# rodrigo-paganini/kalman-vae

Hardware: AMD Instinct MI355X
Metric: sequences/sec (ELBO training step, 32x32xT bouncing-ball) (higher is better)
Workload: dtype f32; 1 GPU; BASELINE configs[1] (configs[2] per-GPU shard): bouncing-ball 32x32, T=50, batch=256/GPU, dynamics=lstm K=3, z=4, u=4, a=2, full train step (fwd incl. sigmoid(x_logits) + loss incl. active-unit stats + bwd + clip + Adam); both the GPU leg and the cpu_baseline leg do this work; preset=c2, global_batch=256, seq_len=50, parallelism=dp1, capture=hipgraph, loss_finite=True, dist_backend=none

## Files before the change

### kalman-vae_amd/csrc/kvae_vae.hip

```cpp
#include <hip/hip_runtime.h>

#include <stdint.h>
#include <stdio.h>
#include <stdlib.h>
#include <string.h>

#include "../../include/kvae_lgssm.h"

namespace kvae {}
using namespace kvae;

extern "C" int kvae_launch_status(const char *what);
static int launch_status(const char *what) { return kvae_launch_status(what); }

#include "vae_epilogue.h"

__device__ __forceinline__ void colsum_v4_body(const float *__restrict__ partials, float *__restrict__ out, int64_t rows, int64_t cols,
                                               unsigned block) {
  __shared__ float4 red[8][64];
  const int lane = threadIdx.x & 63, wv = threadIdx.x >> 6;
  const int64_t c = ((int64_t)block * 64 + lane) * 4;
  float4 s0 = make_float4(0.f, 0.f, 0.f, 0.f), s1 = s0, s2 = s0, s3 = s0;
  if (c < cols) {
    const float *p = partials + c;
// ... 193 lines not shown
}

constexpr int CA_BLOCKS = 512;
constexpr int CA_MAX_SEG = 1024;
__global__ __launch_bounds__(256) void k_grad_sumsq(const float *__restrict__ g, int64_t n, const int32_t *__restrict__ seg_of,
                                                    int n_seg, const float *__restrict__ seg_active,
                                                    const float *__restrict__ div_dev, float *__restrict__ seg_steps,
                                                    float *__restrict__ ws) {
  __shared__ float red[256];
  const float inv = div_dev ? 1.0f / fmaxf(*div_dev, 1.0f) : 1.0f;
  const bool gated = seg_of && seg_active;
  float s = 0.f;
  for (int64_t i = (int64_t)blockIdx.x * 256 + threadIdx.x; i < n; i += (int64_t)gridDim.x * 256) {
    float v = g[i] * inv;
    if (gated && seg_active[seg_of[i]] == 0.f) v = 0.f;
    s = fmaf(v, v, s);
  }
  red[threadIdx.x] = s;
  __syncthreads();
  for (int o = 128; o > 0; o >>= 1) {
    if ((int)threadIdx.x < o) red[threadIdx.x] += red[threadIdx.x + o];
    __syncthreads();
  }
  if (threadIdx.x == 0) ws[blockIdx.x] = red[0];
  if (blockIdx.x == 0)
    for (int sg = threadIdx.x; sg < n_seg; sg += 256)
      if (!seg_active || seg_active[sg] != 0.f) seg_steps[sg] += 1.0f;
}
__global__ __launch_bounds__(256) void k_clip_adam(float *__restrict__ p, const float *__restrict__ g, float *__restrict__ m,
                                                   float *__restrict__ v, int64_t n, const int32_t *__restrict__ seg_of, int n_seg,
                                                   const float *__restrict__ seg_active, const float *__restrict__ seg_steps,
                                                   const float *__restrict__ lr_dev, float lr, float beta1, float beta2, float eps,
                                                   float wd, float clip, const float *__restrict__ div_dev,
                                                   float *__restrict__ norm_out, const float *__restrict__ ws, int nparts) {
  __shared__ float red[256];
  __shared__ float s_step_size[CA_MAX_SEG], s_bc2s[CA_MAX_SEG];
  float s = 0.f;
  for (int i = threadIdx.x; i < nparts; i += 256) s += ws[i];
  red[threadIdx.x] = s;
  const float lrv = lr_dev ? *lr_dev : lr;
  for (int sg = threadIdx.x; sg < n_seg; sg += 256) {
    const float step = seg_steps[sg];
    const bool on = !seg_active || seg_active[sg] != 0.f;
    s_step_size[sg] = on ? lrv / (1.0f - powf(beta1, step)) : -1.0f;
    s_bc2s[sg] = on ? sqrtf(1.0f - powf(beta2, step)) : 1.0f;
  }
  __syncthreads();
  for (int o = 128; o > 0; o >>= 1) {
    if ((int)threadIdx.x < o) red[threadIdx.x] += red[threadIdx.x + o];
    __syncthreads();
  }
  const float total = sqrtf(red[0]);
  if (norm_out && blockIdx.x == 0 && threadIdx.x == 0) *norm_out = total;
  const float inv = div_dev ? 1.0f / fmaxf(*div_dev, 1.0f) : 1.0f;
  const float scale = inv * (clip > 0.f ? fminf(clip / (total + 1e-6f), 1.0f) : 1.0f);
  for (int64_t i = (int64_t)blockIdx.x * 256 + threadIdx.x; i < n; i += (int64_t)gridDim.x * 256) {
    const int sg = seg_of ? seg_of[i] : 0;
    const float step_size = s_step_size[sg], bc2s = s_bc2s[sg];
    if (step_size < 0.f) continue;
    float gi = g[i] * scale;
    const float pi = p[i];
    if (wd != 0.f) gi = fmaf(wd, pi, gi);
    const float mi = m[i] + (gi - m[i]) * (1.0f - beta1);
    const float vi = beta2 * v[i] + (1.0f - beta2) * gi * gi;
    m[i] = mi, v[i] = vi;
    p[i] = pi - step_size * mi / (sqrtf(vi) / bc2s + eps);
  }
}
extern "C" int kvae_clip_adam(float *params, const float *grads, float *exp_avg, float *exp_avg_sq, int64_t n,
                              const int32_t *seg_of, int32_t n_seg, const float *seg_active, float *seg_steps, const float *lr_dev,
                              float lr, float beta1, float beta2, float eps, float weight_decay, float clip, const float *div_dev,
                              float *norm_out, float *ws, void *stream) {
  if (!params || !grads || !exp_avg || !exp_avg_sq || !seg_steps || !ws) return KVAE_ERR_NULL;
  if (n < 1 || n_seg < 1 || n_seg > CA_MAX_SEG || (!seg_of && n_seg != 1)) return KVAE_ERR_ARG;
  const int64_t want = (n + 1023) / 1024;
  const unsigned parts = (unsigned)(want < CA_BLOCKS ? want : CA_BLOCKS);
  k_grad_sumsq<<<dim3(parts), dim3(256), 0, (hipStream_t)stream>>>(grads, n, seg_of, n_seg, seg_active, div_dev, seg_steps, ws);
  int rc = launch_status("k_grad_sumsq");
  if (rc) return rc;
  const unsigned blocks = (unsigned)((n + 255) / 256 < 2048 ? (n + 255) / 256 : 2048);
  k_clip_adam<<<dim3(blocks), dim3(256), 0, (hipStream_t)stream>>>(params, grads, exp_avg, exp_avg_sq, n, seg_of, n_seg, seg_active,
                                                                   seg_steps, lr_dev, lr, beta1, beta2, eps, weight_decay, clip,
                                                                   div_dev, norm_out, ws, (int)parts);
  return launch_status("k_clip_adam");
}

#include "vae_loss.h"

__global__ __launch_bounds__(256) void k_vae_bce_fwd(const float *__restrict__ logits, const float *__restrict__ x,
                                                     float *__restrict__ frame_ll, int64_t frames, int pixels) {
  const int64_t f = (int64_t)blockIdx.x * 4 + (threadIdx.x >> 6);
  const int lane = threadIdx.x & 63;
  if (f >= frames) return;
  const float *l = logits + f * pixels, *t = x + f * pixels;
  float acc = 0.f;
  if ((pixels & 3) == 0 && (((uintptr_t)l | (uintptr_t)t) & 15) == 0) {
    for (int i = lane * 4; i < pixels; i += 256) {
      const float4 a = *reinterpret_cast<const float4 *>(l + i), b = *reinterpret_cast<const float4 *>(t + i);
      acc += bce_logit(a.x, b.x) + bce_logit(a.y, b.y) + bce_logit(a.z, b.z) + bce_logit(a.w, b.w);
    }
  } else {
    for (int i = lane; i < pixels; i += 64) acc += bce_logit(l[i], t[i]);
  }
  for (int off = 32; off > 0; off >>= 1) acc += __shfl_down(acc, off, 64);
  if (lane == 0) frame_ll[f] = -acc;
}

__global__ __launch_bounds__(256) void k_vae_bce_bwd(const float *__restrict__ logits, const float *__restrict__ x,
                                                     const float *__restrict__ g_frame, float *__restrict__ g_logits,
                                                     int64_t total, int pixels) {
  for (int64_t i = ((int64_t)blockIdx.x * 256 + threadIdx.x) * 4; i < total; i += (int64_t)gridDim.x * 1024) {
    const float g = -g_frame[i / pixels];
    const float4 a = *reinterpret_cast<const float4 *>(logits + i), b = *reinterpret_cast<const float4 *>(x + i);
    *reinterpret_cast<float4 *>(g_logits + i) = make_float4(g * (sigmoid_stable(a.x) - b.x), g * (sigmoid_stable(a.y) - b.y),
                                                            g * (sigmoid_stable(a.z) - b.z), g * (sigmoid_stable(a.w) - b.w));
  }
}
__global__ __launch_bounds__(256) void k_vae_bce_bwd_scalar(const float *logits, const float *x, const float *g_frame,
                                                            float *g_logits, int64_t total, int pixels) {
  for (int64_t i = (int64_t)blockIdx.x * 256 + threadIdx.x; i < total; i += (int64_t)gridDim.x * 256)
    g_logits[i] = -g_frame[i / pixels] * (sigmoid_stable(logits[i]) - x[i]);
}

extern "C" {
int kvae_bce_frames_fwd(const float *logits, const float *x, float *frame_ll, int64_t frames, int32_t pixels, void *stream) {
  if (!logits || !x || !frame_ll) return KVAE_ERR_NULL;
  if (frames < 1 || pixels < 1) return KVAE_ERR_ARG;
  k_vae_bce_fwd<<<dim3((unsigned)((frames + 3) / 4)), dim3(256), 0, (hipStream_t)stream>>>(logits, x, frame_ll, frames, pixels);
  return launch_status("k_vae_bce_fwd");
}
int kvae_bce_frames_bwd(const float *logits, const float *x, const float *g_frame, float *g_logits, int64_t frames,
                        int32_t pixels, void *stream) {
  if (!logits || !x || !g_frame || !g_logits) return KVAE_ERR_NULL;
  if (frames < 1 || pixels < 1) return KVAE_ERR_ARG;
  const int64_t total = frames * pixels;
  const bool v4 = (pixels & 3) == 0 && ((((uintptr_t)logits | (uintptr_t)x | (uintptr_t)g_logits) & 15) == 0);
  if (v4)
    k_vae_bce_bwd<<<dim3(epi_grid(total / 4)), dim3(256), 0, (hipStream_t)stream>>>(logits, x, g_frame, g_logits, total, pixels);
  else
    k_vae_bce_bwd_scalar<<<dim3(epi_grid(total)), dim3(256), 0, (hipStream_t)stream>>>(logits, x, g_frame, g_logits, total, pixels);
  return launch_status("k_vae_bce_bwd");
}
}

#include "vae_conv_edge.h"
extern "C" {
int64_t kvae_conv_edge_partial_rows(int64_t N) { return N < 1024 ? (N < 1 ? 1 : N) : 1024; }

int kvae_dec_head_fwd(const float *in, const float *W, const float *bias, float *logits, float *w_scratch, int64_t N,
                      int32_t Cin, int32_t side, void *stream) {
  if (!in || !W || !bias || !logits || !w_scratch) return KVAE_ERR_NULL;
  if (N < 1) return KVAE_ERR_ARG;
  if (Cin != DH_CI || side != DH_S) return KVAE_ERR_DIMS;
  k_dec_head_prep<<<dim3(1), dim3(256), 0, (hipStream_t)stream>>>(W, w_scratch);
  k_dec_head_fwd<<<dim3((unsigned)N), dim3(256), 0, (hipStream_t)stream>>>(in, w_scratch, bias, logits);
  return launch_status("k_dec_head_fwd");
}
int kvae_dec_head_bwd(const float *in, const float *W, const float *g_logits, float *g_in, float *w_partials,
                      float *b_partials, float *w_scratch, int64_t N, int32_t Cin, int32_t side, void *stream) {
  if (!in || !W || !g_logits || !w_partials || !b_partials || !w_scratch) return KVAE_ERR_NULL;
  if (N < 1) return KVAE_ERR_ARG;
  if (Cin != DH_CI || side != DH_S) return KVAE_ERR_DIMS;
  if (g_in) {
    k_dec_head_prep<<<dim3(1), dim3(256), 0, (hipStream_t)stream>>>(W, w_scratch);
    k_dec_head_bwd_data<<<dim3((unsigned)N), dim3(256), 0, (hipStream_t)stream>>>(g_logits, w_scratch, g_in);
    const int rc = launch_status("k_dec_head_bwd_data");
    if (rc) return rc;
  }
  k_dec_head_wrw<<<dim3((unsigned)kvae_conv_edge_partial_rows(N)), dim3(256), 0, (hipStream_t)stream>>>(in, g_logits, w_partials,
                                                                                                     b_partials, N);
  return launch_status("k_dec_head_wrw");
}
int kvae_enc_stem_fwd(const float *x, const float *W, const float *bias, float *out, uint32_t *relu_bits, int64_t N, int32_t Cout,
                      int32_t side, void *stream) {
  if (!x || !W || !bias || !out) return KVAE_ERR_NULL;
  if (N < 1) return KVAE_ERR_ARG;
  if (Cout != ES_CO || side != ES_IN) return KVAE_ERR_DIMS;
  k_enc_stem_fwd<<<dim3((unsigned)N), dim3(256), 0, (hipStream_t)stream>>>(x, W, bias, out, relu_bits);
  return launch_status("k_enc_stem_fwd");
}
int kvae_enc_stem_bwd(const float *x, const float *out, const uint32_t *relu_bits, const float *g_out, float *w_partials,
                      float *b_partials, int64_t N, int32_t Cout, int32_t side, void *stream) {
  if (!x || (!out && !relu_bits) || !g_out || !w_partials || !b_partials) return KVAE_ERR_NULL;
  if (N < 1) return KVAE_ERR_ARG;
  if (Cout != ES_CO || side != ES_IN) return KVAE_ERR_DIMS;
  static const int mfma = getenv("KVAE_STEM_MFMA") ? atoi(getenv("KVAE_STEM_MFMA")) : 1;
  const dim3 grid((unsigned)kvae_conv_edge_partial_rows(N));
  if (mfma == 1 && relu_bits) k_enc_stem_wrw_mfma<true><<<grid, dim3(256), 0, (hipStream_t)stream>>>(x, out, relu_bits, g_out, w_partials, b_partials, N);
  else if (!out) return KVAE_ERR_NULL;
  else if (mfma) k_enc_stem_wrw_mfma<false><<<grid, dim3(256), 0, (hipStream_t)stream>>>(x, out, relu_bits, g_out, w_partials, b_partials, N);
  else k_enc_stem_wrw<<<grid, dim3(256), 0, (hipStream_t)stream>>>(x, out, g_out, w_partials, b_partials, N);
  return launch_status("k_enc_stem_wrw");
}
}

#include "vae_conv_mid.h"
static inline int64_t enc_mid_grid(int64_t N, int32_t side) {
  const int64_t fpi = side == 16 ? 2 : 8, iters = (N + fpi - 1) / fpi;
  return iters < 256 ? (iters < 1 ? 1 : iters) : 256;
}
extern "C" {
int64_t kvae_enc_mid_partial_rows(int64_t N, int32_t side) { return enc_mid_grid(N, side); }

int kvae_enc_mid_fwd(const float *in, const float *W, const float *bias, float *out, int64_t N, int32_t C, int32_t side,
                     void *stream) {
  if (!in || !W || !bias || !out) return KVAE_ERR_NULL;
  if (N < 1 || (N + 256 * 8) * EM_C * side * side * 4 >= EM_MAX_BYTES) return KVAE_ERR_ARG;
  if (C != EM_C || (side != 16 && side != 8)) return KVAE_ERR_DIMS;
  const dim3 grid((unsigned)enc_mid_grid(N, side));
  if (side == 16) k_enc_mid_fwd<16><<<grid, dim3(256), 0, (hipStream_t)stream>>>(in, W, bias, out, N);
  else k_enc_mid_fwd<8><<<grid, dim3(256), 0, (hipStream_t)stream>>>(in, W, bias, out, N);
  return launch_status("k_enc_mid_fwd");
}
int kvae_enc_mid_bwd(const float *in, const float *W, const float *out, const float *g_out, float *g_in,
                     float *w_partials, float *b_partials, int64_t N, int32_t C, int32_t side, void *stream) {
  if (!in || !W || !out || !g_out || !w_partials || !b_partials) return KVAE_ERR_NULL;
  if (N < 1 || (N + 256 * 8) * EM_C * side * side * 4 >= EM_MAX_BYTES) return KVAE_ERR_ARG;
  if (C != EM_C || (side != 16 && side != 8)) return KVAE_ERR_DIMS;
  const dim3 grid((unsigned)enc_mid_grid(N, side));
  if (g_in) {
    if (side == 16) k_enc_mid_bwd_data<16><<<grid, dim3(256), 0, (hipStream_t)stream>>>(W, out, g_out, g_in, N);
    else k_enc_mid_bwd_data<8><<<grid, dim3(256), 0, (hipStream_t)stream>>>(W, out, g_out, g_in, N);
    const int rc = launch_status("k_enc_mid_bwd_data");
    if (rc) return rc;
  }
  if (side == 16) k_enc_mid_wrw<16><<<grid, dim3(256), 0, (hipStream_t)stream>>>(in, out, g_out, w_partials, b_partials, N);
  else k_enc_mid_wrw<8><<<grid, dim3(256), 0, (hipStream_t)stream>>>(in, out, g_out, w_partials, b_partials, N);
  return launch_status("k_enc_mid_wrw");
}
}

#include "vae_conv_up_wino.h"
static bool dec_up_wino() {
  static const int env = getenv("KVAE_WINO") ? atoi(getenv("KVAE_WINO")) : 1;
  return env != 0;
}
static int g_dec_up_wgs = 0;
static inline int64_t dec_up_cap() {
  static const int env = getenv("KVAE_UP_WGS") ? atoi(getenv("KVAE_UP_WGS")) : 0;
  const int v = env >= 1 && env <= 256 ? env : __atomic_load_n(&g_dec_up_wgs, __ATOMIC_RELAXED);
  return v >= 1 && v <= 256 ? v : 256;
}
static inline int64_t dec_up_grid(int64_t N, int32_t side) {
  const int64_t fpi = side == 8 ? 2 : 8, iters = (N + fpi - 1) / fpi, cap = dec_up_cap();
  return iters < cap ? (iters < 1 ? 1 : iters) : cap;
}
extern "C" {
int64_t kvae_dec_up_partial_rows(int64_t N, int32_t side) { return dec_up_grid(N, side); }
int32_t kvae_dec_up_set_workgroups(int32_t n) {
  const int32_t prev = (int32_t)dec_up_cap();
  __atomic_store_n(&g_dec_up_wgs, n >= 1 && n <= 256 ? n : 0, __ATOMIC_RELAXED);
  return prev;
}

int kvae_dec_up_fwd(const float *x, const float *W, const float *bias, float *out, int64_t N, int32_t Cin, int32_t side,
                    void *stream) {
  if (!x || !W || !bias || !out) return KVAE_ERR_NULL;
  if (N < 1 || (N + 256 * 8) * UP_CO * side * side * 4 >= EM_MAX_BYTES) return KVAE_ERR_ARG;
  if (Cin != UP_CI || (side != 8 && side != 4)) return KVAE_ERR_DIMS;
  const dim3 grid((unsigned)dec_up_grid(N, side));
  if (dec_up_wino()) {
    const int64_t sets = side == 8 ? N : (N + 3) / 4;
    const dim3 wgrid((unsigned)(sets < dec_up_cap() ? sets : dec_up_cap()));
    if (side == 8) k_dec_up_fwd_wino<8><<<wgrid, dim3(512), 0, (hipStream_t)stream>>>(x, W, bias, out, N);
    else k_dec_up_fwd_wino<4><<<wgrid, dim3(512), 0, (hipStream_t)stream>>>(x, W, bias, out, N);
    return launch_status("k_dec_up_fwd_wino");
  }
  if (side == 8) k_dec_up_fwd<8><<<grid, dim3(256), 0, (hipStream_t)stream>>>(x, W, bias, out, N);
  else k_dec_up_fwd<4><<<grid, dim3(256), 0, (hipStream_t)stream>>>(x, W, bias, out, N);
  return launch_status("k_dec_up_fwd");
}
int kvae_dec_up_bwd(const float *x, const float *W, const float *out, const float *g_out, float *g_x, float *w_partials,
                    float *b_partials, int64_t N, int32_t Cin, int32_t side, void *stream) {
  if (!x || !W || !out || !g_out || !w_partials || !b_partials) return KVAE_ERR_NULL;
  if (N < 1 || (N + 256 * 8) * UP_CO * side * side * 4 >= EM_MAX_BYTES) return KVAE_ERR_ARG;
  if (Cin != UP_CI || (side != 8 && side != 4)) return KVAE_ERR_DIMS;
  const dim3 grid((unsigned)dec_up_grid(N, side));
  if (g_x) {
    const int64_t sets = side == 8 ? N : (N + 3) / 4;
    const dim3 wgrid((unsigned)(sets < dec_up_cap() ? sets : dec_up_cap()));
    if (dec_up_wino() && side == 8) k_dec_up_bwd_data_wino<8><<<wgrid, dim3(512), 0, (hipStream_t)stream>>>(W, out, g_out, g_x, N);
    else if (dec_up_wino()) k_dec_up_bwd_data_wino<4><<<wgrid, dim3(512), 0, (hipStream_t)stream>>>(W, out, g_out, g_x, N);
    else if (side == 8) k_dec_up_bwd_data<8><<<grid, dim3(256), 0, (hipStream_t)stream>>>(W, out, g_out, g_x, N);
    else k_dec_up_bwd_data<4><<<grid, dim3(256), 0, (hipStream_t)stream>>>(W, out, g_out, g_x, N);
    const int rc = launch_status("k_dec_up_bwd_data");
    if (rc) return rc;
  }
  if (dec_up_wino()) {
    if (side == 8) k_dec_up_wrw_wino<8><<<grid, dim3(512), 0, (hipStream_t)stream>>>(x, out, g_out, w_partials, b_partials, N);
    else k_dec_up_wrw_wino<4><<<grid, dim3(512), 0, (hipStream_t)stream>>>(x, out, g_out, w_partials, b_partials, N);
    return launch_status("k_dec_up_wrw_wino");
  }
  if (side == 8) k_dec_up_wrw<8><<<grid, dim3(256), 0, (hipStream_t)stream>>>(x, out, g_out, w_partials, b_partials, N);
  else k_dec_up_wrw<4><<<grid, dim3(256), 0, (hipStream_t)stream>>>(x, out, g_out, w_partials, b_partials, N);
  return launch_status("k_dec_up_wrw");
}
}

#include "vae_heads.h"
extern "C" {
int64_t kvae_head_partial_rows(void) { return HD_WAVES; }

int kvae_enc_head_fwd(const float *feat, const float *Wmu, const float *bmu, const float *Wvar, const float *bvar,
                      const float *eps, float *mu, float *var, float *a, int64_t N, int32_t F, int32_t A,
                      float noise_emission, void *stream) {
  if (!feat || !Wmu || !bmu || !Wvar || !bvar || !mu || !var || !a) return KVAE_ERR_NULL;
  if (N < 1) return KVAE_ERR_ARG;
  if (F != HD_F || A != HD_A) return KVAE_ERR_DIMS;
// ... 61 lines not shown
```

### kalman-vae_amd/csrc/vae_conv_edge.h

```cpp
#pragma once
#include <hip/hip_runtime.h>
#include <stdint.h>

namespace kvae {

constexpr int DH_CI = 32, DH_CO = 4, DH_S = 16, DH_TS = 18, DH_CS = 325;
constexpr int DH_W = DH_CO * DH_CI * 9;
typedef float kv_f2 __attribute__((ext_vector_type(2)));
typedef float kv_f4 __attribute__((ext_vector_type(4)));

__global__ __launch_bounds__(256) void k_dec_head_prep(const float *__restrict__ W, float *__restrict__ scratch) {
  for (int i = threadIdx.x; i < DH_W; i += 256) {
    const int co = i / (DH_CI * 9), r = i - co * DH_CI * 9, ci = r / 9, k = r - ci * 9;
    const float w = W[i];
    scratch[(ci * 9 + k) * DH_CO + co] = w;
    scratch[DH_W + (co * 9 + k) * DH_CI + ci] = w;
  }
}

__device__ __forceinline__ void dh_zero_halo(float *tile, int channels) {
  for (int i = threadIdx.x; i < channels * 68; i += 256) {
    const int c = i / 68, j = i - c * 68;
    int r, q;
    if (j < 18) { r = 0; q = j; }
    else if (j < 36) { r = 17; q = j - 18; }
    else if (j < 52) { r = j - 35; q = 0; }
    else { r = j - 51; q = 17; }
    tile[c * DH_CS + r * DH_TS + q] = 0.f;
  }
}
__device__ __forceinline__ void dh_store_interior(float *tile, int i, const float4 v) {
  const int e = i * 4, ci = e >> 8, hw = e & 255, h = hw >> 4, w = hw & 15;
  float *d = tile + ci * DH_CS + (h + 1) * DH_TS + (w + 1);
  d[0] = v.x; d[1] = v.y; d[2] = v.z; d[3] = v.w;
}

__global__ __launch_bounds__(256) void k_dec_head_fwd(const float *__restrict__ in, const float *__restrict__ scratch,
                                                      const float *__restrict__ bias, float *__restrict__ logits) {
  __shared__ float tile[DH_CI * 256];
  const int64_t n = blockIdx.x;
  const float4 *src = reinterpret_cast<const float4 *>(in + n * DH_CI * 256);
  float4 pre[8];
#pragma unroll
  for (int j = 0; j < 8; ++j) pre[j] = src[threadIdx.x + 256 * j];
#pragma unroll
  for (int j = 0; j < 8; ++j) reinterpret_cast<float4 *>(tile)[threadIdx.x + 256 * j] = pre[j];
  __syncthreads();
  const int h = threadIdx.x >> 4, w = threadIdx.x & 15;
  constexpr int OOB = 1 << 24;
  const int tb = (h - 1) * 16 + (w - 1);
  int base[9];
#pragma unroll
  for (int tap = 0; tap < 9; ++tap) {
    const int ky = tap / 3, kx = tap % 3;
    const bool z = (ky == 0 && h == 0) || (ky == 2 && h == 15) || (kx == 0 && w == 0) || (kx == 2 && w == 15);
    base[tap] = (z ? OOB : tb) + ky * 16 + kx;
  }
  kv_f2 a01 = {bias[0], bias[1]}, a23 = {bias[2], bias[3]};
  const kv_f4 *Wf = reinterpret_cast<const kv_f4 *>(scratch);
#pragma unroll 4
  for (int ci = 0; ci < DH_CI; ++ci) {
#pragma unroll
    for (int tap = 0; tap < 9; ++tap) {
      const float v = tile[base[tap] + ci * 256];
      const kv_f4 wv = Wf[ci * 9 + tap];
      a01 += wv.xy * v;
      a23 += wv.zw * v;
    }
  }
  float *o = logits + n * 1024 + (2 * h) * 32 + 2 * w;
  *reinterpret_cast<float2 *>(o) = make_float2(a01.x, a01.y);
  *reinterpret_cast<float2 *>(o + 32) = make_float2(a23.x, a23.y);
}

__global__ __launch_bounds__(256) void k_dec_head_bwd_data(const float *__restrict__ g_logits,
                                                           const float *__restrict__ scratch, float *__restrict__ g_in) {
  __shared__ float gt[DH_CO * DH_CS];
  const int64_t n = blockIdx.x;
  float gp[4];
#pragma unroll
  for (int j = 0; j < 4; ++j) gp[j] = g_logits[n * 1024 + threadIdx.x + 256 * j];
  dh_zero_halo(gt, DH_CO);
#pragma unroll
  for (int j = 0; j < 4; ++j) {
    const int i = threadIdx.x + 256 * j, oh = i >> 5, ow = i & 31, co = (oh & 1) * 2 + (ow & 1);
    gt[co * DH_CS + ((oh >> 1) + 1) * DH_TS + (ow >> 1) + 1] = gp[j];
  }
  __syncthreads();
  const int h = threadIdx.x >> 4, w = threadIdx.x & 15;
  kv_f2 acc[DH_CI / 2];
#pragma unroll
  for (int j = 0; j < DH_CI / 2; ++j) acc[j] = kv_f2{0.f, 0.f};
  const kv_f2 *Wb = reinterpret_cast<const kv_f2 *>(scratch + DH_W);
#pragma unroll
  for (int co = 0; co < DH_CO; ++co)
#pragma unroll
    for (int ky = 0; ky < 3; ++ky)
#pragma unroll
      for (int kx = 0; kx < 3; ++kx) {
        const float v = gt[co * DH_CS + (h + 2 - ky) * DH_TS + (w + 2 - kx)];
        const kv_f2 *wr = Wb + (co * 9 + ky * 3 + kx) * (DH_CI / 2);
#pragma unroll
        for (int j = 0; j < DH_CI / 2; ++j) acc[j] += wr[j] * v;
      }
  float *o = g_in + n * DH_CI * 256 + threadIdx.x;
#pragma unroll
  for (int j = 0; j < DH_CI / 2; ++j) {
    o[(2 * j) * 256] = acc[j].x;
    o[(2 * j + 1) * 256] = acc[j].y;
  }
}

__global__ __launch_bounds__(256) void k_dec_head_wrw(const float *__restrict__ in, const float *__restrict__ g_logits,
                                                      float *__restrict__ partial, float *__restrict__ partial_b, int64_t N) {
  constexpr int CS = 257, OOB = 1 << 24;
  __shared__ float lds[DH_CI * CS + DH_CO * 256];
  __shared__ float redb[8 * DH_CO];
  float *tile = lds, *gt = lds + DH_CI * CS;
  const int ci = threadIdx.x & 31, grp = threadIdx.x >> 5;
  const int tin = (((threadIdx.x & 63) >> 4) << 6) | ((threadIdx.x >> 6) << 4) | (threadIdx.x & 15);
  kv_f2 acc[DH_CO / 2][9];
  float accb[DH_CO];
#pragma unroll
  for (int c = 0; c < DH_CO / 2; ++c)
#pragma unroll
    for (int k = 0; k < 9; ++k) acc[c][k] = kv_f2{0.f, 0.f};
#pragma unroll
  for (int co = 0; co < DH_CO; ++co) accb[co] = 0.f;
  float4 pre[8];
  float gp[4];
  int64_t n = blockIdx.x;
  if (n < N) {
    const float4 *src = reinterpret_cast<const float4 *>(in + n * DH_CI * 256);
#pragma unroll
    for (int j = 0; j < 8; ++j) pre[j] = src[tin + 256 * j];
#pragma unroll
    for (int j = 0; j < 4; ++j) gp[j] = g_logits[n * 1024 + threadIdx.x + 256 * j];
  }
  for (; n < N; n += gridDim.x) {
    __syncthreads();
#pragma unroll
    for (int j = 0; j < 8; ++j) {
      const int e = (tin + 256 * j) * 4;
      float *d = tile + (e >> 8) * CS + (e & 255);
      d[0] = pre[j].x; d[1] = pre[j].y; d[2] = pre[j].z; d[3] = pre[j].w;
    }
#pragma unroll
    for (int j = 0; j < 4; ++j) {
      const int i = threadIdx.x + 256 * j, oh = i >> 5, ow = i & 31, co = (oh & 1) * 2 + (ow & 1);
      gt[co * 256 + (oh >> 1) * 16 + (ow >> 1)] = gp[j];
    }
    __syncthreads();
    const int64_t nn = n + gridDim.x;
    if (nn < N) {
      const float4 *src = reinterpret_cast<const float4 *>(in + nn * DH_CI * 256);
#pragma unroll
      for (int j = 0; j < 8; ++j) pre[j] = src[tin + 256 * j];
#pragma unroll
      for (int j = 0; j < 4; ++j) gp[j] = g_logits[nn * 1024 + threadIdx.x + 256 * j];
    }
#pragma unroll
    for (int rr = 0; rr < 2; ++rr) {
      const int h = 2 * grp + rr;
      int rb[3];
#pragma unroll
      for (int ky = 0; ky < 3; ++ky) {
        const bool off = (ky == 0 && rr == 0 && grp == 0) || (ky == 2 && rr == 1 && grp == 7);
        rb[ky] = (off ? OOB : ci * CS) + (h + ky - 1) * 16;
      }
      float c0[3] = {0.f, 0.f, 0.f}, c1[3], c2[3];
#pragma unroll
      for (int ky = 0; ky < 3; ++ky) c1[ky] = tile[rb[ky]];
#pragma unroll
      for (int w = 0; w < 16; ++w) {
#pragma unroll
        for (int ky = 0; ky < 3; ++ky) c2[ky] = w + 1 < 16 ? tile[rb[ky] + w + 1] : 0.f;
        const int hw = h * 16 + w;
        const kv_f2 g01 = {gt[hw], gt[256 + hw]}, g23 = {gt[512 + hw], gt[768 + hw]};
        accb[0] += g01.x; accb[1] += g01.y; accb[2] += g23.x; accb[3] += g23.y;
#pragma unroll
        for (int ky = 0; ky < 3; ++ky) {
          acc[0][ky * 3 + 0] += g01 * c0[ky]; acc[1][ky * 3 + 0] += g23 * c0[ky];
          acc[0][ky * 3 + 1] += g01 * c1[ky]; acc[1][ky * 3 + 1] += g23 * c1[ky];
          acc[0][ky * 3 + 2] += g01 * c2[ky]; acc[1][ky * 3 + 2] += g23 * c2[ky];
          c0[ky] = c1[ky];
          c1[ky] = c2[ky];
        }
      }
    }
  }
  __syncthreads();
  float *red = lds;
#pragma unroll
  for (int k = 0; k < 9; ++k) {
    float *r = red + (grp * 32 + ci) * 36 + k;
    r[0] = acc[0][k].x; r[9] = acc[0][k].y; r[18] = acc[1][k].x; r[27] = acc[1][k].y;
  }
  if (ci == 0) {
#pragma unroll
    for (int co = 0; co < DH_CO; ++co) redb[grp * 4 + co] = accb[co];
  }
  __syncthreads();
  for (int o = threadIdx.x; o < DH_W; o += 256) {
    const int co = o / (DH_CI * 9), r = o - co * DH_CI * 9, c2 = r / 9, k = r - c2 * 9;
    float s = 0.f;
    for (int gq = 0; gq < 8; ++gq) s += red[(gq * 32 + c2) * 36 + co * 9 + k];
    partial[(int64_t)blockIdx.x * DH_W + o] = s;
  }
  if (threadIdx.x < DH_CO) {
    float s = 0.f;
    for (int gq = 0; gq < 8; ++gq) s += redb[gq * 4 + threadIdx.x];
    partial_b[(int64_t)blockIdx.x * DH_CO + threadIdx.x] = s;
  }
}


constexpr int ES_CO = 32, ES_IN = 32, ES_OUT = 16, ES_TS = 35;

__device__ __forceinline__ void es_load_tile(float *tile, const float *__restrict__ x) {
  for (int i = threadIdx.x; i < 34 * ES_TS; i += 256) tile[i] = 0.f;
  __syncthreads();
  const float4 v = reinterpret_cast<const float4 *>(x)[threadIdx.x];
  const int e = threadIdx.x * 4, h = e >> 5, w = e & 31;
  float *d = tile + (h + 1) * ES_TS + (w + 1);
  d[0] = v.x; d[1] = v.y; d[2] = v.z; d[3] = v.w;
}

__global__ __launch_bounds__(256) void k_enc_stem_fwd(const float *__restrict__ x, const float *__restrict__ W,
                                                      const float *__restrict__ bias, float *__restrict__ out,
                                                      uint32_t *__restrict__ relu_bits) {
  __shared__ float tile[34 * ES_TS];
  const int64_t n = blockIdx.x;
  es_load_tile(tile, x + n * 1024);
  __syncthreads();
  const int oh = threadIdx.x >> 4, ow = threadIdx.x & 15;
  float v[9];
#pragma unroll
  for (int ky = 0; ky < 3; ++ky)
#pragma unroll
    for (int kx = 0; kx < 3; ++kx) v[ky * 3 + kx] = tile[(2 * oh + ky) * ES_TS + 2 * ow + kx];
  float *o = out + n * ES_CO * 256 + threadIdx.x;
  uint32_t bits = 0;
#pragma unroll 8
  for (int co = 0; co < ES_CO; ++co) {
    float acc = bias[co];
#pragma unroll
    for (int k = 0; k < 9; ++k) acc = fmaf(W[co * 9 + k], v[k], acc);
    o[co * 256] = fmaxf(acc, 0.f);
    bits |= (acc > 0.f ? 1u : 0u) << co;
  }
  if (relu_bits) relu_bits[n * 256 + threadIdx.x] = bits;
}

__global__ __launch_bounds__(256) void k_enc_stem_wrw(const float *__restrict__ x, const float *__restrict__ out,
                                                      const float *__restrict__ g_out, float *__restrict__ partial,
                                                      float *__restrict__ partial_b, int64_t N) {
  __shared__ float tile[34 * ES_TS];
  __shared__ float gt[ES_CO * 257];
  const int co = threadIdx.x & 31, grp = threadIdx.x >> 5;
  float acc[9], accb = 0.f;
#pragma unroll
  for (int k = 0; k < 9; ++k) acc[k] = 0.f;
  for (int64_t n = blockIdx.x; n < N; n += gridDim.x) {
    __syncthreads();
    es_load_tile(tile, x + n * 1024);
    const float4 *g4 = reinterpret_cast<const float4 *>(g_out + n * ES_CO * 256);
    const float4 *o4 = reinterpret_cast<const float4 *>(out + n * ES_CO * 256);
    for (int i = threadIdx.x; i < ES_CO * 64; i += 256) {
      const float4 gv = g4[i], ov = o4[i];
      const int e = i * 4, c = e >> 8, hw = e & 255;
      float *d = gt + c * 257 + hw;
      d[0] = ov.x > 0.f ? gv.x : 0.f; d[1] = ov.y > 0.f ? gv.y : 0.f;
      d[2] = ov.z > 0.f ? gv.z : 0.f; d[3] = ov.w > 0.f ? gv.w : 0.f;
    }
    __syncthreads();
    for (int i = 0; i < 32; ++i) {
      const int hw = grp * 32 + i, oh = hw >> 4, ow = hw & 15;
      const float gv = gt[co * 257 + hw];
      accb += gv;
      const float *t = tile + (2 * oh) * ES_TS + 2 * ow;
#pragma unroll
      for (int ky = 0; ky < 3; ++ky)
#pragma unroll
        for (int kx = 0; kx < 3; ++kx) acc[ky * 3 + kx] = fmaf(gv, t[ky * ES_TS + kx], acc[ky * 3 + kx]);
    }
  }
  __syncthreads();
  float *red = gt;
#pragma unroll
  for (int k = 0; k < 9; ++k) red[(grp * 32 + co) * 10 + k] = acc[k];
  red[(grp * 32 + co) * 10 + 9] = accb;
  __syncthreads();
  for (int o = threadIdx.x; o < ES_CO * 10; o += 256) {
    const int c = o / 10, k = o - c * 10;
    float s = 0.f;
    for (int gq = 0; gq < 8; ++gq) s += red[(gq * 32 + c) * 10 + k];
    if (k < 9) partial[(int64_t)blockIdx.x * (ES_CO * 9) + c * 9 + k] = s;
    else partial_b[(int64_t)blockIdx.x * ES_CO + c] = s;
  }
}

typedef float es_f4 __attribute__((ext_vector_type(4)));
template <bool BITS>
__global__ __launch_bounds__(256) void k_enc_stem_wrw_mfma(const float *__restrict__ x, const float *__restrict__ out,
                                                           const uint32_t *__restrict__ relu_bits, const float *__restrict__ g_out,
                                                           float *__restrict__ partial,
                                                           float *__restrict__ partial_b, int64_t N) {
  __shared__ float tile[34 * ES_TS];
  constexpr int GS = 260;
  __shared__ __attribute__((aligned(16))) float gt[ES_CO * GS];
  __shared__ __attribute__((aligned(16))) uint32_t mw[256];
  const int lane = threadIdx.x & 63, wv = threadIdx.x >> 6, j = lane & 15, g = lane >> 4;
  const int tap = j < 9 ? j : 8;
  const float *tb = tile + (8 * wv) * ES_TS + 2 * g + (tap / 3) * ES_TS + tap % 3;
  const float *ga = gt + j * GS + 64 * wv + g;
  es_f4 acc0 = {0.f, 0.f, 0.f, 0.f}, acc1 = acc0;
  float4 gv[8], ov[8], xv;
  uint32_t mv = 0;
  auto fetch = [&](int64_t n) {
    const bool ok = n < N;
    const float4 *g4 = reinterpret_cast<const float4 *>(g_out + (ok ? n : 0) * ES_CO * 256);
    const float4 *o4 = reinterpret_cast<const float4 *>(out + (ok ? n : 0) * ES_CO * 256);
#pragma unroll
    for (int q = 0; q < 8; ++q) {
      gv[q] = g4[threadIdx.x + 256 * q];
      if constexpr (!BITS) ov[q] = o4[threadIdx.x + 256 * q];
    }
    xv = reinterpret_cast<const float4 *>(x + (ok ? n : 0) * 1024)[threadIdx.x];
    if constexpr (BITS) mv = relu_bits[(ok ? n : 0) * 256 + threadIdx.x];
  };
  fetch(blockIdx.x);
  for (int i = threadIdx.x; i < 34 * ES_TS; i += 256) tile[i] = 0.f;
  for (int64_t n = blockIdx.x; n < N; n += gridDim.x) {
    __syncthreads();
    {
      float *d = tile + ((threadIdx.x >> 3) + 1) * ES_TS + 4 * (threadIdx.x & 7) + 1;
      d[0] = xv.x; d[1] = xv.y; d[2] = xv.z; d[3] = xv.w;
    }
    if constexpr (BITS) {
      mw[threadIdx.x] = mv;
      __syncthreads();
    }
#pragma unroll
    for (int q = 0; q < 8; ++q) {
      const int e = (threadIdx.x + 256 * q) * 4, c = e >> 8, hw = e & 255;
      float4 md;
      if constexpr (BITS) {
        const uint4 m = *reinterpret_cast<const uint4 *>(mw + hw);
        md = make_float4((m.x >> c) & 1u ? gv[q].x : 0.f, (m.y >> c) & 1u ? gv[q].y : 0.f, (m.z >> c) & 1u ? gv[q].z : 0.f,
                         (m.w >> c) & 1u ? gv[q].w : 0.f);
      } else {
        md = make_float4(ov[q].x > 0.f ? gv[q].x : 0.f, ov[q].y > 0.f ? gv[q].y : 0.f, ov[q].z > 0.f ? gv[q].z : 0.f,
                         ov[q].w > 0.f ? gv[q].w : 0.f);
      }
      *reinterpret_cast<float4 *>(gt + c * GS + hw) = md;
    }
    __syncthreads();
    fetch(n + gridDim.x);
#pragma unroll
    for (int s = 0; s < 16; ++s) {
      const float xb = tb[2 * (s >> 2) * ES_TS + 8 * (s & 3)];
      const float b = j == 9 ? 1.0f : xb;
      acc0 = __builtin_amdgcn_mfma_f32_16x16x4f32(ga[4 * s], b, acc0, 0, 0, 0);
      acc1 = __builtin_amdgcn_mfma_f32_16x16x4f32(ga[16 * GS + 4 * s], b, acc1, 0, 0, 0);
    }
// ... 19 lines not shown
```

Baseline: 96080 sequences/s.

## Move decoder head conv forward and weight-gradient onto 4x4x1 f32 MFMA

Rewrites the decoder head 3x3 conv forward as a persistent grid-strided kernel. It reads weights into registers directly, dropping the separate prep launch, and computes outputs with mfma_f32_4x4x1f32 plus an LDS cross-wave fold. The weight-gradient kernel is likewise rebuilt on 4x4x1 MFMA, using buffer loads, staged prefetch and a new reduction layout. The prep kernel now writes only the transposed half still used by bwd_data. The goal is to move FP32 FMA work onto matrix cores and cut launch and LDS overhead, at the cost of more complex indexing and higher register and LDS pressure.

New measurement: 95090 sequences/s. 0.99x the previous value.

```diff
diff --git a/kalman-vae_amd/csrc/kvae_vae.hip b/kalman-vae_amd/csrc/kvae_vae.hip
--- a/kalman-vae_amd/csrc/kvae_vae.hip
+++ b/kalman-vae_amd/csrc/kvae_vae.hip
@@ -369,8 +369,7 @@
   if (!in || !W || !bias || !logits || !w_scratch) return KVAE_ERR_NULL;
   if (N < 1) return KVAE_ERR_ARG;
   if (Cin != DH_CI || side != DH_S) return KVAE_ERR_DIMS;
-  k_dec_head_prep<<<dim3(1), dim3(256), 0, (hipStream_t)stream>>>(W, w_scratch);
-  k_dec_head_fwd<<<dim3((unsigned)N), dim3(256), 0, (hipStream_t)stream>>>(in, w_scratch, bias, logits);
+  k_dec_head_fwd<<<dim3((unsigned)(N < DHF_GRID ? N : DHF_GRID)), dim3(256), 0, (hipStream_t)stream>>>(in, W, bias, logits, N);
   return launch_status("k_dec_head_fwd");
 }
 int kvae_dec_head_bwd(const float *in, const float *W, const float *g_logits, float *g_in, float *w_partials,
diff --git a/kalman-vae_amd/csrc/vae_conv_edge.h b/kalman-vae_amd/csrc/vae_conv_edge.h
--- a/kalman-vae_amd/csrc/vae_conv_edge.h
+++ b/kalman-vae_amd/csrc/vae_conv_edge.h
@@ -12,9 +12,7 @@
 __global__ __launch_bounds__(256) void k_dec_head_prep(const float *__restrict__ W, float *__restrict__ scratch) {
   for (int i = threadIdx.x; i < DH_W; i += 256) {
     const int co = i / (DH_CI * 9), r = i - co * DH_CI * 9, ci = r / 9, k = r - ci * 9;
-    const float w = W[i];
-    scratch[(ci * 9 + k) * DH_CO + co] = w;
-    scratch[DH_W + (co * 9 + k) * DH_CI + ci] = w;
+    scratch[DH_W + (co * 9 + k) * DH_CI + ci] = W[i];
   }
 }
 
@@ -35,42 +33,77 @@
   d[0] = v.x; d[1] = v.y; d[2] = v.z; d[3] = v.w;
 }
 
-__global__ __launch_bounds__(256) void k_dec_head_fwd(const float *__restrict__ in, const float *__restrict__ scratch,
-                                                      const float *__restrict__ bias, float *__restrict__ logits) {
-  __shared__ float tile[DH_CI * 256];
-  const int64_t n = blockIdx.x;
-  const float4 *src = reinterpret_cast<const float4 *>(in + n * DH_CI * 256);
-  float4 pre[8];
-#pragma unroll
-  for (int j = 0; j < 8; ++j) pre[j] = src[threadIdx.x + 256 * j];
-#pragma unroll
-  for (int j = 0; j < 8; ++j) reinterpret_cast<float4 *>(tile)[threadIdx.x + 256 * j] = pre[j];
-  __syncthreads();
-  const int h = threadIdx.x >> 4, w = threadIdx.x & 15;
+constexpr int DHF_PS = 18 * 16;
+constexpr int DHF_GRID = 768;
+__global__ __launch_bounds__(256) void k_dec_head_fwd(const float *__restrict__ in, const float *__restrict__ W,
+                                                         const float *__restrict__ bias, float *__restrict__ logits, int64_t N) {
+  __shared__ __attribute__((aligned(16))) float tile[DH_CI * DHF_PS];
+  __shared__ __attribute__((aligned(16))) float fold[4 * 1024];
+  const int tid = threadIdx.x, lane = tid & 63, wv = tid >> 6;
+  for (int i = tid; i < DH_CI * 32; i += 256) tile[(i >> 5) * DHF_PS + ((i & 16) ? 17 * 16 : 0) + (i & 15)] = 0.f;
+  float wr[8][9];
+  {
+    const float *wp = W + ((lane & 3) * DH_CI + 8 * wv) * 9;
+#pragma unroll
+    for (int cl = 0; cl < 8; ++cl)
+#pragma unroll
+      for (int k = 0; k < 9; ++k) wr[cl][k] = wp[cl * 9 + k];
+  }
   constexpr int OOB = 1 << 24;
-  const int tb = (h - 1) * 16 + (w - 1);
-  int base[9];
-#pragma unroll
-  for (int tap = 0; tap < 9; ++tap) {
-    const int ky = tap / 3, kx = tap % 3;
-    const bool z = (ky == 0 && h == 0) || (ky == 2 && h == 15) || (kx == 0 && w == 0) || (kx == 2 && w == 15);
-    base[tap] = (z ? OOB : tb) + ky * 16 + kx;
-  }
-  kv_f2 a01 = {bias[0], bias[1]}, a23 = {bias[2], bias[3]};
-  const kv_f4 *Wf = reinterpret_cast<const kv_f4 *>(scratch);
-#pragma unroll 4
-  for (int ci = 0; ci < DH_CI; ++ci) {
-#pragma unroll
-    for (int tap = 0; tap < 9; ++tap) {
-      const float v = tile[base[tap] + ci * 256];
-      const kv_f4 wv = Wf[ci * 9 + tap];
-      a01 += wv.xy * v;
-      a23 += wv.zw * v;
-    }
-  }
-  float *o = logits + n * 1024 + (2 * h) * 32 + 2 * w;
-  *reinterpret_cast<float2 *>(o) = make_float2(a01.x, a01.y);
-  *reinterpret_cast<float2 *>(o + 32) = make_float2(a23.x, a23.y);
+  const int q = lane & 3;
+  const int mid = 8 * wv * DHF_PS + (lane >> 2) * 16 + 4 * q;
+  const int left = q == 0 ? OOB : mid - 1, right = q == 3 ? OOB : mid + 4;
+  kv_f4 b0 = {0.f, 0.f, 0.f, 0.f};
+  if (wv == 0) b0 = kv_f4{bias[0], bias[1], bias[2], bias[3]};
+  const int hh = tid >> 4, ww = tid & 15;
+  const int ru = (ww & 3) * 64 + ((hh * 4 + (ww >> 2)) ^ (4 * (ww & 3)));
+  kv_f4 pre[8];
+  int64_t n = blockIdx.x;
+  if (n < N) {
+    const kv_f4 *src = reinterpret_cast<const kv_f4 *>(in + n * DH_CI * 256);
+#pragma unroll
+    for (int j = 0; j < 8; ++j) pre[j] = src[tid + 256 * j];
+  }
+  for (; n < N; n += gridDim.x) {
+#pragma unroll
+    for (int j = 0; j < 8; ++j) reinterpret_cast<kv_f4 *>(tile)[(wv + 4 * j) * (DHF_PS / 4) + 4 + lane] = pre[j];
+    __syncthreads();
+    const int64_t nn = n + gridDim.x;
+    if (nn < N) {
+      const kv_f4 *src = reinterpret_cast<const kv_f4 *>(in + nn * DH_CI * 256);
+#pragma unroll
+      for (int j = 0; j < 8; ++j) pre[j] = src[tid + 256 * j];
+    }
+    kv_f4 acc[4] = {b0, b0, b0, b0};
+#pragma unroll
+    for (int cl = 0; cl < 8; ++cl) {
+      float win[3][6];
+#pragma unroll
+      for (int ky = 0; ky < 3; ++ky) {
+        const kv_f4 m = *reinterpret_cast<const kv_f4 *>(tile + mid + cl * DHF_PS + ky * 16);
+        win[ky][0] = tile[left + cl * DHF_PS + ky * 16];
+        win[ky][1] = m.x; win[ky][2] = m.y; win[ky][3] = m.z; win[ky][4] = m.w;
+        win[ky][5] = tile[right + cl * DHF_PS + ky * 16];
+      }
+#pragma unroll
+      for (int ky = 0; ky < 3; ++ky)
+#pragma unroll
+        for (int kx = 0; kx < 3; ++kx)
+#pragma unroll
+          for (int p = 0; p < 4; ++p) acc[p] = __builtin_amdgcn_mfma_f32_4x4x1f32(wr[cl][ky * 3 + kx], win[ky][p + kx], acc[p], 0, 0, 0);
+    }
+#pragma unroll
+    for (int p = 0; p < 4; ++p) reinterpret_cast<kv_f4 *>(fold)[wv * 256 + p * 64 + (lane ^ (4 * p))] = acc[p];
+    __syncthreads();
+    const kv_f4 *fu = reinterpret_cast<const kv_f4 *>(fold) + ru;
+    kv_f4 s = fu[0];
+    s += fu[256];
+    s += fu[512];
+    s += fu[768];
+    float *o = logits + n * 1024 + (2 * hh) * 32 + 2 * ww;
+    *reinterpret_cast<float2 *>(o) = make_float2(s.x, s.y);
+    *reinterpret_cast<float2 *>(o + 32) = make_float2(s.z, s.w);
+  }
 }
 
 __global__ __launch_bounds__(256) void k_dec_head_bwd_data(const float *__restrict__ g_logits,
@@ -111,106 +144,121 @@
   }
 }
 
-__global__ __launch_bounds__(256) void k_dec_head_wrw(const float *__restrict__ in, const float *__restrict__ g_logits,
-                                                      float *__restrict__ partial, float *__restrict__ partial_b, int64_t N) {
-  constexpr int CS = 257, OOB = 1 << 24;
-  __shared__ float lds[DH_CI * CS + DH_CO * 256];
-  __shared__ float redb[8 * DH_CO];
-  float *tile = lds, *gt = lds + DH_CI * CS;
-  const int ci = threadIdx.x & 31, grp = threadIdx.x >> 5;
-  const int tin = (((threadIdx.x & 63) >> 4) << 6) | ((threadIdx.x >> 6) << 4) | (threadIdx.x & 15);
-  kv_f2 acc[DH_CO / 2][9];
-  float accb[DH_CO];
-#pragma unroll
-  for (int c = 0; c < DH_CO / 2; ++c)
-#pragma unroll
-    for (int k = 0; k < 9; ++k) acc[c][k] = kv_f2{0.f, 0.f};
-#pragma unroll
-  for (int co = 0; co < DH_CO; ++co) accb[co] = 0.f;
-  float4 pre[8];
+constexpr int DHW_PS = 264;
+__global__ __launch_bounds__(256, 4) void k_dec_head_wrw(const float *__restrict__ in, const float *__restrict__ g_logits,
+                                                         float *__restrict__ partial, float *__restrict__ partial_b, int64_t N) {
+  constexpr int OOB = 1 << 24;
+  __shared__ __attribute__((aligned(16))) float lds[(DH_CI + DH_CO) * DHW_PS];
+  __shared__ float redb[16 * DH_CO];
+  float *tile = lds, *gt = lds + DH_CI * DHW_PS;
+  const int tid = threadIdx.x, lane = tid & 63, wv = __builtin_amdgcn_readfirstlane(tid >> 6), w = lane >> 2, j = lane & 3;
+  const int frames = (int)N;
+  const int pb = (8 * wv + j) * DHW_PS + w;
+  const int bL = w == 0 ? OOB : pb - 1, bM = pb, bR = w == 15 ? OOB : pb + 1;
+  const int ga = j * DHW_PS + w;
+  kv_f4 acc[2][9];
+#pragma unroll
+  for (int gi = 0; gi < 2; ++gi)
+#pragma unroll
+    for (int k = 0; k < 9; ++k) acc[gi][k] = kv_f4{0.f, 0.f, 0.f, 0.f};
+  float accb = 0.f;
+  const int dp = (8 * wv) * (DHW_PS / 4) + lane;
+  const uint32_t so = ((8 * wv) * 64 + lane) * 16, go = tid * 4;
+  const int gw = (((tid >> 5) & 1) * 2 + (tid & 1)) * DHW_PS + (tid >> 6) * 16 + ((tid & 31) >> 1);
+  auto frame_rsrc = [](const float *p, int bytes) {
+    return __builtin_amdgcn_make_buffer_rsrc(const_cast<float *>(p), 0, bytes, 0x00020000);
+  };
+  auto ld4 = [](__amdgpu_buffer_rsrc_t r, uint32_t off, int soff) {
+    typedef uint32_t u4 __attribute__((ext_vector_type(4)));
+    const u4 v = __builtin_amdgcn_raw_buffer_load_b128(r, off, soff, 0);
+    return kv_f4{__uint_as_float(v.x), __uint_as_float(v.y), __uint_as_float(v.z), __uint_as_float(v.w)};
+  };
+  kv_f4 pre[4];
   float gp[4];
-  int64_t n = blockIdx.x;
-  if (n < N) {
-    const float4 *src = reinterpret_cast<const float4 *>(in + n * DH_CI * 256);
-#pragma unroll
-    for (int j = 0; j < 8; ++j) pre[j] = src[tin + 256 * j];
-#pragma unroll
-    for (int j = 0; j < 4; ++j) gp[j] = g_logits[n * 1024 + threadIdx.x + 256 * j];
-  }
-  for (; n < N; n += gridDim.x) {
-    __syncthreads();
-#pragma unroll
-    for (int j = 0; j < 8; ++j) {
-      const int e = (tin + 256 * j) * 4;
-      float *d = tile + (e >> 8) * CS + (e & 255);
-      d[0] = pre[j].x; d[1] = pre[j].y; d[2] = pre[j].z; d[3] = pre[j].w;
-    }
-#pragma unroll
-    for (int j = 0; j < 4; ++j) {
-      const int i = threadIdx.x + 256 * j, oh = i >> 5, ow = i & 31, co = (oh & 1) * 2 + (ow & 1);
-      gt[co * 256 + (oh >> 1) * 16 + (ow >> 1)] = gp[j];
-    }
-    __syncthreads();
-    const int64_t nn = n + gridDim.x;
-    if (nn < N) {
-      const float4 *src = reinterpret_cast<const float4 *>(in + nn * DH_CI * 256);
-#pragma unroll
-      for (int j = 0; j < 8; ++j) pre[j] = src[tin + 256 * j];
-#pragma unroll
-      for (int j = 0; j < 4; ++j) gp[j] = g_logits[nn * 1024 + threadIdx.x + 256 * j];
-    }
-#pragma unroll
-    for (int rr = 0; rr < 2; ++rr) {
-      const int h = 2 * grp + rr;
-      int rb[3];
-#pragma unroll
-      for (int ky = 0; ky < 3; ++ky) {
-        const bool off = (ky == 0 && rr == 0 && grp == 0) || (ky == 2 && rr == 1 && grp == 7);
-        rb[ky] = (off ? OOB : ci * CS) + (h + ky - 1) * 16;
+  int n = blockIdx.x;
+  if (n < frames) {
+    const __amdgpu_buffer_rsrc_t ri = frame_rsrc(in + (int64_t)n * DH_CI * 256, DH_CI * 1024), rg = frame_rsrc(g_logits + (int64_t)n * 1024, 4096);
+#pragma unroll
+    for (int q = 0; q < 4; ++q) gp[q] = __uint_as_float(__builtin_amdgcn_raw_buffer_load_b32(rg, go, q * 1024, 0));
+#pragma unroll
+    for (int gi = 0; gi < 2; ++gi) {
+#pragma unroll
+      for (int q = 0; q < 4; ++q) pre[q] = ld4(ri, so, gi * 4096 + q * 1024);
+#pragma unroll
+      for (int q = 0; q < 4; ++q) reinterpret_cast<kv_f4 *>(tile)[dp + (4 * gi + q) * (DHW_PS / 4)] = pre[q];
+    }
+  }
+  for (; n < frames; n += gridDim.x) {
+    __syncthreads();
+#pragma unroll
+    for (int q = 0; q < 4; ++q) gt[gw + 64 * q] = gp[q];
+    __syncthreads();
+    const int nn = n + (int)gridDim.x;
+    const bool more = nn < frames;
+    const __amdgpu_buffer_rsrc_t ri = frame_rsrc(in + (int64_t)nn * DH_CI * 256, DH_CI * 1024), rg = frame_rsrc(g_logits + (int64_t)nn * 1024, 4096);
+    if (more) {
+#pragma unroll
+      for (int q = 0; q < 4; ++q) pre[q] = ld4(ri, so, q * 1024);
+    }
+#pragma unroll
+    for (int gi = 0; gi < 2; ++gi) {
+      float a0 = 0.f, a1 = gt[ga], a2 = 0.f;
+#pragma unroll
+      for (int r = 0; r < 16; ++r) {
+        if (r + 1 < 16) a2 = gt[ga + (r + 1) * 16];
+        if (gi == 0) accb += a1;
+        const int o = gi * 4 * DHW_PS + r * 16;
+        const float vL = tile[bL + o], vM = tile[bM + o], vR = tile[bR + o];
+        if (r + 1 < 16) {
+          acc[gi][0] = __builtin_amdgcn_mfma_f32_4x4x1f32(a2, vL, acc[gi][0], 0, 0, 0);
+          acc[gi][1] = __builtin_amdgcn_mfma_f32_4x4x1f32(a2, vM, acc[gi][1], 0, 0, 0);
+          acc[gi][2] = __builtin_amdgcn_mfma_f32_4x4x1f32(a2, vR, acc[gi][2], 0, 0, 0);
+        }
+        acc[gi][3] = __builtin_amdgcn_mfma_f32_4x4x1f32(a1, vL, acc[gi][3], 0, 0, 0);
+        acc[gi][4] = __builtin_amdgcn_mfma_f32_4x4x1f32(a1, vM, acc[gi][4], 0, 0, 0);
+        acc[gi][5] = __builtin_amdgcn_mfma_f32_4x4x1f32(a1, vR, acc[gi][5], 0, 0, 0);
+        if (r > 0) {
+          acc[gi][6] = __builtin_amdgcn_mfma_f32_4x4x1f32(a0, vL, acc[gi][6], 0, 0, 0);
+          acc[gi][7] = __builtin_amdgcn_mfma_f32_4x4x1f32(a0, vM, acc[gi][7], 0, 0, 0);
+          acc[gi][8] = __builtin_amdgcn_mfma_f32_4x4x1f32(a0, vR, acc[gi][8], 0, 0, 0);
+        }
+        a0 = a1;
+        a1 = a2;
       }
-      float c0[3] = {0.f, 0.f, 0.f}, c1[3], c2[3];
-#pragma unroll
-      for (int ky = 0; ky < 3; ++ky) c1[ky] = tile[rb[ky]];
-#pragma unroll
-      for (int w = 0; w < 16; ++w) {
-#pragma unroll
-        for (int ky = 0; ky < 3; ++ky) c2[ky] = w + 1 < 16 ? tile[rb[ky] + w + 1] : 0.f;
-        const int hw = h * 16 + w;
-        const kv_f2 g01 = {gt[hw], gt[256 + hw]}, g23 = {gt[512 + hw], gt[768 + hw]};
-        accb[0] += g01.x; accb[1] += g01.y; accb[2] += g23.x; accb[3] += g23.y;
-#pragma unroll
-        for (int ky = 0; ky < 3; ++ky) {
-          acc[0][ky * 3 + 0] += g01 * c0[ky]; acc[1][ky * 3 + 0] += g23 * c0[ky];
-          acc[0][ky * 3 + 1] += g01 * c1[ky]; acc[1][ky * 3 + 1] += g23 * c1[ky];
-          acc[0][ky * 3 + 2] += g01 * c2[ky]; acc[1][ky * 3 + 2] += g23 * c2[ky];
-          c0[ky] = c1[ky];
-          c1[ky] = c2[ky];
+      if (more) {
+#pragma unroll
+        for (int q = 0; q < 4; ++q) reinterpret_cast<kv_f4 *>(tile)[dp + (4 * gi + q) * (DHW_PS / 4)] = pre[q];
+        if (gi == 0) {
+#pragma unroll
+          for (int q = 0; q < 4; ++q) pre[q] = ld4(ri, so, 4096 + q * 1024);
+        } else {
+#pragma unroll
+          for (int q = 0; q < 4; ++q) gp[q] = __uint_as_float(__builtin_amdgcn_raw_buffer_load_b32(rg, go, q * 1024, 0));
         }
       }
     }
   }
-  __syncthreads();
   float *red = lds;
-#pragma unroll
-  for (int k = 0; k < 9; ++k) {
-    float *r = red + (grp * 32 + ci) * 36 + k;
-    r[0] = acc[0][k].x; r[9] = acc[0][k].y; r[18] = acc[1][k].x; r[27] = acc[1][k].y;
-  }
-  if (ci == 0) {
-#pragma unroll
-    for (int co = 0; co < DH_CO; ++co) redb[grp * 4 + co] = accb[co];
-  }
-  __syncthreads();
-  for (int o = threadIdx.x; o < DH_W; o += 256) {
-    const int co = o / (DH_CI * 9), r = o - co * DH_CI * 9, c2 = r / 9, k = r - c2 * 9;
+  const int l2 = __builtin_amdgcn_mbcnt_hi(~0u, __builtin_amdgcn_mbcnt_lo(~0u, 0u)), t2 = wv * 64 + l2;
+  const int rw = (l2 >> 2) * 576 + wv * 144 + (l2 & 3) * 36;
+#pragma unroll
+  for (int gi = 0; gi < 2; ++gi) {
+    __syncthreads();
+#pragma unroll
+    for (int k = 0; k < 9; ++k) *reinterpret_cast<kv_f4 *>(red + rw + k * 4) = acc[gi][k];
+    if (gi == 0 && wv == 0) redb[l2] = accb;
+    __syncthreads();
+    for (int o = t2; o < 576; o += 256) {
+      float s = 0.f;
+      for (int c = 0; c < 16; ++c) s += red[c * 576 + o];
+      const int ci = 4 * (2 * (o / 144) + gi) + (o % 144) / 36, k = (o % 36) >> 2, co = o & 3;
+      partial[(int64_t)blockIdx.x * DH_W + (co * DH_CI + ci) * 9 + k] = s;
+    }
+  }
+  if (t2 < DH_CO) {
     float s = 0.f;
-    for (int gq = 0; gq < 8; ++gq) s += red[(gq * 32 + c2) * 36 + co * 9 + k];
-    partial[(int64_t)blockIdx.x * DH_W + o] = s;
-  }
-  if (threadIdx.x < DH_CO) {
-    float s = 0.f;
-    for (int gq = 0; gq < 8; ++gq) s += redb[gq * 4 + threadIdx.x];
-    partial_b[(int64_t)blockIdx.x * DH_CO + threadIdx.x] = s;
+    for (int c = 0; c < 16; ++c) s += redb[c * DH_CO + t2];
+    partial_b[(int64_t)blockIdx.x * DH_CO + t2] = s;
   }
 }
 
```
